# PravCoder/Multi-Modal-Medical-Imaging-and-Report-ML-Diagnosis-System

Measured on AMD Instinct MI355X. Metric: multimodal samples/sec (train fwd+bwd) at 1/2/4/8 MI355X; MFMA util %, higher is better.
Workload: dtype bf16; 1 GPU; C4: ResNet-50 + 2-layer BiLSTM, 128 samples/GPU (1024 global at 8 GPUs); image_tower=resnet50, text_tower=bilstm, global_batch=128, per_gpu_batch=128, seq_len=128, image_hw=224, parallelism=dp1

## Files before the change

### multi-modal-medical-imaging-and-report-ml-diagnosis-system_amd/csrc/capi.cpp

```cpp
#include <stdarg.h>
#include <stdio.h>
#include <stdlib.h>

#include <mutex>
#include <vector>

#include <hip/hip_ext.h>

#include "../../include/mmdx.h"
#include "common.h"

static thread_local char g_err[512] = "";

extern "C" void mmdx_set_error(const char* fmt, ...) {
  va_list ap;
  va_start(ap, fmt);
  vsnprintf(g_err, sizeof(g_err), fmt, ap);
  va_end(ap);
}

extern "C" const char* mmdx_last_error(void) { return g_err; }

extern "C" int mmdx_version(void) { return 1; }

namespace mmdx {

static long env_long(const char* name, long dflt) {
  const char* e = getenv(name);
  return e && *e ? atol(e) : dflt;
}

static Knobs read_knobs() {
  Knobs k;
  const long w = env_long("MMDX_CONV_N64_WIDE", -1);
  k.conv_n64_wide = w < 0 ? -1 : w == 0 ? 0 : 1;
  k.conv_8w128 = env_long("MMDX_CONV_8W128", 1) != 0;
  k.stem_direct = env_long("MMDX_STEM_DIRECT", 1) != 0;
  const long t = env_long("MMDX_WGRAD_TARGET", 256);
  k.wgrad_target = t >= 64 && t <= 4096 ? t : 256;
  k.wgrad_rq = env_long("MMDX_WGRAD_RQ", 1) != 0;
  k.gemm256_fwd_min = env_long("MMDX_GEMM256_FWD_MIN", 90);
  k.gemm_8w128 = env_long("MMDX_GEMM_8W128", 1) != 0;
  const long s = env_long("MMDX_SPLITK_TARGET", 256);
  k.splitk_target = s >= 64 ? s : 256;
  k.splitk_vec = env_long("MMDX_SPLITK_VEC", 1) != 0;
  k.wgrad_bias_fused = env_long("MMDX_WGRAD_BIAS_FUSED", 1) != 0;
  k.bias_grad_gemm = env_long("MMDX_BIAS_GRAD_GEMM", 0) == 1;
  k.ln_bwd_rpw = env_long("MMDX_LN_BWD_RPW", 8) == 4 ? 4 : 8;
  k.attn_fwd_nw = (int)env_long("MMDX_ATTN_FWD_NW", 0);
  k.attn_bwd_nw = (int)env_long("MMDX_ATTN_BWD_NW", 0);
  k.lstm_bwd_probe = env_long("MMDX_LSTM_BWD_PROBE", 0) != 0;
  k.bn_bwd_pair = env_long("MMDX_BN_BWD_PAIR", 1) != 0;
  return k;
}

static Knobs g_knobs;
static std::once_flag g_knobs_once;

const Knobs& knobs() {
  std::call_once(g_knobs_once, [] { g_knobs = read_knobs(); });
  return g_knobs;
}

}

extern "C" int mmdx_reload_config(void) {
  mmdx::knobs();
  mmdx::g_knobs = mmdx::read_knobs();
  return 0;
}

extern "C" int mmdx_bn_bwd_pair_enabled(void) { return mmdx::knobs().bn_bwd_pair ? 1 : 0; }

extern "C" int mmdx_stream_create(int priority, int cus, void** out) {
  MMDX_CHECK_ARG(out, "mmdx_stream_create: out is NULL");
  *out = nullptr;
  int dev = 0, n = 0;
  MMDX_CHECK_ARG(hipGetDevice(&dev) == hipSuccess &&
                     hipDeviceGetAttribute(&n, hipDeviceAttributeMultiprocessorCount, dev) ==
                         hipSuccess && n > 0,
                 "mmdx_stream_create: no device");
  hipStream_t s = nullptr;
  if (cus <= 0 || cus >= n) {
    MMDX_CHECK_ARG(hipStreamCreateWithPriority(&s, hipStreamNonBlocking, priority) == hipSuccess,
                   "mmdx_stream_create: hipStreamCreateWithPriority failed");
  } else {
    std::vector<uint32_t> mask((n + 31) / 32, 0u);
    for (int i = 0; i < cus; ++i) {
      const int cu = (int)((long)i * n / cus);
      mask[cu / 32] |= 1u << (cu % 32);
    }
    MMDX_CHECK_ARG(hipExtStreamCreateWithCUMask(&s, (uint32_t)mask.size(), mask.data()) ==
                       hipSuccess,
                   "mmdx_stream_create: hipExtStreamCreateWithCUMask failed");
  }
  *out = (void*)s;
  return 0;
}

extern "C" int mmdx_stream_destroy(void* s) {
  MMDX_CHECK_ARG(s && hipStreamDestroy((hipStream_t)s) == hipSuccess, "mmdx_stream_destroy");
  return 0;
}
```

### multi-modal-medical-imaging-and-report-ml-diagnosis-system_amd/csrc/common.h

```cpp
#pragma once
#include <hip/hip_runtime.h>

#include <algorithm>
#include <stdint.h>
#include <stddef.h>

namespace mmdx {

typedef __bf16 bf16;
typedef _Float16 f16;
typedef __attribute__((ext_vector_type(8))) __bf16 bf16x8;
typedef __attribute__((ext_vector_type(8))) _Float16 f16x8;
typedef __attribute__((ext_vector_type(4))) __bf16 bf16x4;
typedef __attribute__((ext_vector_type(4))) float f32x4;
typedef __attribute__((ext_vector_type(2))) float f32x2;
typedef __attribute__((ext_vector_type(16))) float f32x16;
typedef __attribute__((ext_vector_type(4))) unsigned int u32x4;
typedef __attribute__((ext_vector_type(4))) short s16x4;

enum Dtype { F32 = 0, BF16 = 1, F16 = 2 };
enum Act { ACT_NONE = 0, ACT_RELU = 1, ACT_GELU = 2, ACT_GELU_BWD = 3 };

constexpr int WAVE = 64;

struct Knobs {
  int conv_n64_wide;
  bool conv_8w128;
  bool stem_direct;
  long wgrad_target;
  bool wgrad_rq;
  long gemm256_fwd_min;
  bool gemm_8w128;
  long splitk_target;
  bool splitk_vec;
  bool wgrad_bias_fused;
  bool bias_grad_gemm;
  int ln_bwd_rpw;
  int attn_fwd_nw;
  int attn_bwd_nw;
  bool lstm_bwd_probe;
  bool bn_bwd_pair;
};
const Knobs& knobs();

__device__ __forceinline__ float to_f(float x) { return x; }
__device__ __forceinline__ float to_f(bf16 x) { return (float)x; }
__device__ __forceinline__ float to_f(f16 x) { return (float)x; }
template <typename T> __device__ __forceinline__ T from_f(float x);
template <> __device__ __forceinline__ float from_f<float>(float x) { return x; }
template <> __device__ __forceinline__ bf16 from_f<bf16>(float x) { return (bf16)x; }
template <> __device__ __forceinline__ f16 from_f<f16>(float x) { return (f16)x; }

template <typename T> struct Vec16;
template <> struct Vec16<bf16> { static constexpr int N = 8; typedef bf16x8 type; };
template <> struct Vec16<float> { static constexpr int N = 4; typedef f32x4 type; };
template <> struct Vec16<f16> { static constexpr int N = 8; typedef f16x8 type; };

#define MMDX_DISPATCH(dtype, ...)                  \
  do {                                             \
    if ((dtype) == ::mmdx::BF16) {                 \
      typedef ::mmdx::bf16 T;                      \
      __VA_ARGS__;                                 \
    } else if ((dtype) == ::mmdx::F16) {           \
      typedef ::mmdx::f16 T;                       \
      __VA_ARGS__;                                 \
    } else {                                       \
      typedef float T;                             \
      __VA_ARGS__;                                 \
    }                                              \
  } while (0)

__device__ __forceinline__ float gelu_erf(float x) {
  return 0.5f * x * (1.0f + erff(x * 0.70710678118654752f));
}
__device__ __forceinline__ float gelu_erf_grad(float x) {
  const float cdf = 0.5f * (1.0f + erff(x * 0.70710678118654752f));
  const float pdf = 0.39894228040143268f * __expf(-0.5f * x * x);
  return cdf + x * pdf;
}

__device__ __forceinline__ float wave_sum(float v) {
#pragma unroll
  for (int o = 32; o > 0; o >>= 1) v += __shfl_xor(v, o, 64);
  return v;
}
__device__ __forceinline__ float wave_max(float v) {
#pragma unroll
  for (int o = 32; o > 0; o >>= 1) v = fmaxf(v, __shfl_xor(v, o, 64));
  return v;
}

template <int NT>
__device__ __forceinline__ float block_sum(float v, float* red) {
  v = wave_sum(v);
  const int w = threadIdx.x >> 6, l = threadIdx.x & 63;
  if (l == 0) red[w] = v;
  __syncthreads();
  float t = 0.f;
#pragma unroll
  for (int i = 0; i < NT / 64; ++i) t += red[i];
  __syncthreads();
  return t;
}

static inline int grid_for(long n, int per = 256) {
  return (int)std::max<long>(1, std::min<long>((n + per - 1) / per, 8192));
}

#define GRID_STRIDE(i, n) \
  for (long i = blockIdx.x * (long)blockDim.x + threadIdx.x; i < (n); i += (long)gridDim.x * blockDim.x)

}

extern "C" void mmdx_set_error(const char* fmt, ...);

#define MMDX_CHECK_ARG(cond, ...)                     \
  do {                                               \
    if (!(cond)) {                                   \
      mmdx_set_error(__VA_ARGS__);                   \
      return -22;                       \
    }                                                \
  } while (0)

#define MMDX_LAUNCH_CHECK()                                          \
  do {                                                               \
    hipError_t _e = hipGetLastError();                               \
    if (_e != hipSuccess) {                                          \
      mmdx_set_error("HIP launch failed: %s", hipGetErrorString(_e)); \
      return -(int)_e;                                               \
    }                                                                \
  } while (0)
```

### multi-modal-medical-imaging-and-report-ml-diagnosis-system_amd/csrc/misc.hip

```cpp
#include <algorithm>

#include "common.h"
#include "dropout_rng.h"
#include "pool.h"
#include "../../include/mmdx.h"

namespace mmdx {

template <typename T>
__global__ void maxpool_fwd_kernel(const T* __restrict__ x, int N, int H, int W, int C, int k,
                                   int s, int p, T* __restrict__ y, uint8_t* __restrict__ am,
                                   int P, int Q) {
  typedef typename Vec16<T>::type V;
  constexpr int VEC = Vec16<T>::N;
  const int cv = C / VEC;
  const long total = (long)N * P * Q * cv;
  GRID_STRIDE(i, total) {
    const int c = (int)(i % cv) * VEC;
    long t = i / cv;
    const int q = (int)(t % Q); t /= Q;
    const int pp = (int)(t % P);
    const int n = (int)(t / P);
    float best[VEC];
    int arg[VEC];
// ... 4 lines not shown
      if ((unsigned)ih >= (unsigned)H) continue;
      for (int ss = 0; ss < k; ++ss) {
        const int iw = q * s - p + ss;
        if ((unsigned)iw >= (unsigned)W) continue;
        const V v = *(const V*)(x + (((long)n * H + ih) * W + iw) * C + c);
#pragma unroll
        for (int j = 0; j < VEC; ++j) {
          const float f = to_f(v[j]);
          if (arg[j] < 0 || f > best[j] || (f != f && best[j] == best[j])) {
            best[j] = f;
            arg[j] = r * k + ss;
          }
        }
      }
    }
    V o;
#pragma unroll
    for (int j = 0; j < VEC; ++j) {
      o[j] = from_f<T>(best[j]);
      am[i * VEC + j] = (uint8_t)arg[j];
    }
    *(V*)(y + i * VEC) = o;
  }
}

template <typename T>
__global__ void maxpool_bwd_kernel(const uint8_t* __restrict__ am, const T* __restrict__ dy,
                                   int N, int H, int W, int C, int k, int s, int p, int P, int Q,
                                   T* __restrict__ dx) {
  typedef typename Vec16<T>::type V;
  constexpr int VEC = Vec16<T>::N;
  const int cv = C / VEC;
  const long total = (long)N * H * W * cv;
  GRID_STRIDE(i, total) {
    const int c = (int)(i % cv) * VEC;
    long t = i / cv;
    const int w = (int)(t % W); t /= W;
    const int h = (int)(t % H);
    const int n = (int)(t / H);
    float acc[VEC];
#pragma unroll
    for (int j = 0; j < VEC; ++j) acc[j] = 0.f;
    const int p_lo = max(0, (h + p - k + s) / s), p_hi = min(P - 1, (h + p) / s);
    const int q_lo = max(0, (w + p - k + s) / s), q_hi = min(Q - 1, (w + p) / s);
    for (int pp = p_lo; pp <= p_hi; ++pp) {
      const int r = h + p - pp * s;
      if (r < 0 || r >= k) continue;
      for (int q = q_lo; q <= q_hi; ++q) {
        const int ss = w + p - q * s;
        if (ss < 0 || ss >= k) continue;
        const long o = (((long)n * P + pp) * Q + q) * C + c;
        const V g = *(const V*)(dy + o);
#pragma unroll
        for (int j = 0; j < VEC; ++j)
          if (am[o + j] == r * k + ss) acc[j] += to_f(g[j]);
      }
    }
    V out;
#pragma unroll
    for (int j = 0; j < VEC; ++j) out[j] = from_f<T>(acc[j]);
    *(V*)(dx + i * VEC) = out;
  }
}


__device__ __forceinline__ void bn_coef_fwd(const float* gamma, const float* beta,
                                            const float* mean, const float* rstd, int c,
                                            float& scale, float& shift) {
  const float g = gamma ? gamma[c] : 1.f;
  scale = g * rstd[c];
  shift = (beta ? beta[c] : 0.f) - mean[c] * g * rstd[c];
}

template <typename T, bool BN = false>
__global__ void maxpool3s2_fwd_kernel(const T* __restrict__ x, int N, int H, int W, int C,
                                      int p, T* __restrict__ y, uint8_t* __restrict__ am, int P,
                                      int Q, const float* __restrict__ gamma,
                                      const float* __restrict__ beta,
                                      const float* __restrict__ mean,
                                      const float* __restrict__ rstd, int relu) {
  typedef typename Vec16<T>::type V;
  constexpr int VEC = Vec16<T>::N;
  typedef typename ArgPack<VEC>::type A;
  const int cv = C / VEC;
  const long total = (long)N * P * Q * cv;
  const bool fixed_c = blockDim.x % cv == 0;
  float sc[VEC], sh[VEC];
  if constexpr (BN) {
    if (fixed_c) {
      const int c0 = (int)(threadIdx.x % cv) * VEC;
#pragma unroll
      for (int j = 0; j < VEC; ++j) bn_coef_fwd(gamma, beta, mean, rstd, c0 + j, sc[j], sh[j]);
    }
  }
  GRID_STRIDE(i, total) {
    const unsigned ui = (unsigned)i, ucv = (unsigned)cv;
    const int c = (int)(ui % ucv) * VEC;
    if constexpr (BN) {
      if (!fixed_c) {
#pragma unroll
        for (int j = 0; j < VEC; ++j) bn_coef_fwd(gamma, beta, mean, rstd, c + j, sc[j], sh[j]);
      }
    }
    unsigned t = ui / ucv;
    const int q = (int)(t % (unsigned)Q); t /= (unsigned)Q;
    const int pp = (int)(t % (unsigned)P);
    const int n = (int)(t / (unsigned)P);
    V v[9];
    bool ok[9];
#pragma unroll
    for (int r = 0; r < 3; ++r) {
      const int ih = pp * 2 - p + r;
#pragma unroll
      for (int ss = 0; ss < 3; ++ss) {
        const int iw = q * 2 - p + ss;
        ok[r * 3 + ss] = (unsigned)ih < (unsigned)H && (unsigned)iw < (unsigned)W;
        v[r * 3 + ss] = ok[r * 3 + ss] ? *(const V*)(x + (((long)n * H + ih) * W + iw) * C + c)
                                       : V{};
      }
    }
    float best[VEC];
    int arg[VEC];
#pragma unroll
    for (int j = 0; j < VEC; ++j) { best[j] = -INFINITY; arg[j] = -1; }
#pragma unroll
    for (int w9 = 0; w9 < 9; ++w9) {
      if (!ok[w9]) continue;
#pragma unroll
      for (int j = 0; j < VEC; ++j) {
        float f = to_f(v[w9][j]);
        if constexpr (BN) {
          f = f * sc[j] + sh[j];
          if (relu) f = fmaxf(f, 0.f);
          f = to_f(from_f<T>(f));
        }
        if (arg[j] < 0 || f > best[j] || (f != f && best[j] == best[j])) {
          best[j] = f;
          arg[j] = w9;
        }
      }
    }
    V o;
    A packed = 0;
#pragma unroll
    for (int j = 0; j < VEC; ++j) {
      o[j] = from_f<T>(best[j]);
      packed |= (A)(uint8_t)arg[j] << (8 * j);
    }
    *(A*)(am + i * VEC) = packed;
    *(V*)(y + i * VEC) = o;
  }
}

template <typename T>
__global__ void maxpool3s2_bwd_kernel(const uint8_t* __restrict__ am, const T* __restrict__ dy,
                                      int N, int H, int W, int C, int p, int P, int Q,
                                      T* __restrict__ dx) {
  typedef typename Vec16<T>::type V;
  constexpr int VEC = Vec16<T>::N;
  const Pool3s2Grad<T> pg{am, dy, H, W, C, p, P, Q};
  const int cv = C / VEC;
  const long total = (long)N * H * W * cv;
  GRID_STRIDE(i, total) {
    const unsigned ui = (unsigned)i, ucv = (unsigned)cv;
    const int c = (int)(ui % ucv) * VEC;
    unsigned t = ui / ucv;
    const int w = (int)(t % (unsigned)W); t /= (unsigned)W;
    const int h = (int)(t % (unsigned)H);
    const int n = (int)(t / (unsigned)H);
    *(V*)(dx + i * VEC) = pg.at(n, h, w, c);
  }
}

template <typename T>
__global__ void avgpool_fwd_kernel(const T* __restrict__ x, int N, int HW, int C,
                                   T* __restrict__ y) {
  const long total = (long)N * C;
  GRID_STRIDE(i, total) {
    const int c = (int)(i % C);
    const long n = i / C;
    float acc = 0.f;
    for (int k = 0; k < HW; ++k) acc += to_f(x[(n * HW + k) * C + c]);
    y[i] = from_f<T>(acc / (float)HW);
  }
}

template <typename T>
__global__ void avgpool_bwd_kernel(const T* __restrict__ dy, int N, int HW, int C,
                                   T* __restrict__ dx) {
  const long total = (long)N * HW * C;
  const float inv = 1.f / (float)HW;
  GRID_STRIDE(i, total) {
    const int c = (int)(i % C);
    const long n = i / ((long)HW * C);
    dx[i] = from_f<T>(to_f(dy[n * C + c]) * inv);
  }
}

template <typename T>
__global__ void nchw_to_nhwc_kernel(const float* __restrict__ x, int N, int C, int H, int W,
                                    int cp, T* __restrict__ y) {
  const long total = (long)N * H * W;
  GRID_STRIDE(i, total) {
    const long hw = i % ((long)H * W);
    const long n = i / ((long)H * W);
    for (int c = 0; c < cp; ++c)
      y[i * cp + c] = from_f<T>(c < C ? x[(n * C + c) * H * W + hw] : 0.f);
  }
}

template <typename D, typename S>
__global__ void cast_kernel(const S* __restrict__ x, long n, D* __restrict__ y) {
  GRID_STRIDE(i, n) y[i] = from_f<D>(to_f(x[i]));
}

__global__ void axpby_kernel(long n, float a, const float* __restrict__ x, float b,
                             const float* __restrict__ y, float* __restrict__ out) {
  GRID_STRIDE(i, n) out[i] = a * x[i] + (y ? b * y[i] : 0.f);
}

template <typename T>
__global__ void gelu_bwd_kernel(const T* __restrict__ pre, const T* __restrict__ dy, long n,
                                T* __restrict__ dx) {
  GRID_STRIDE(i, n) dx[i] = from_f<T>(to_f(dy[i]) * gelu_erf_grad(to_f(pre[i])));
}

constexpr int BG_ROWS = 256;
constexpr int BG_ROWS_MIN = 32;
static int bias_grad_rows(long M, int N, int vec) {
  const long nx = (N / vec + 63) / 64;
  const long nb_target = (1024 + nx - 1) / nx;
  long rows = (M + nb_target - 1) / nb_target;
  rows = (rows + 3) / 4 * 4;
  return (int)std::max<long>(BG_ROWS_MIN, std::min<long>(BG_ROWS, rows));
}
template <typename T>
__global__ __launch_bounds__(256) void bias_grad_partial_kernel(const T* __restrict__ dy,
                                                                long M, int N,
                                                                float* __restrict__ part,
                                                                int rows) {
  typedef typename Vec16<T>::type V;
  constexpr int VEC = Vec16<T>::N;
  __shared__ float red[4][64 * VEC];
  const int cv = threadIdx.x & 63, lane = threadIdx.x >> 6;
  const int j = blockIdx.x * 64 + cv;
  const bool ok = j < N / VEC;
  const long r0 = (long)blockIdx.y * rows, r1 = min(M, r0 + rows);
  float acc[VEC];
#pragma unroll
  for (int e = 0; e < VEC; ++e) acc[e] = 0.f;
  if (ok) {
#pragma unroll 4
    for (long r = r0 + lane; r < r1; r += 4) {
      const V v = ((const V*)(dy + r * N))[j];
#pragma unroll
      for (int e = 0; e < VEC; ++e) acc[e] += to_f(v[e]);
    }
  }
#pragma unroll
  for (int e = 0; e < VEC; ++e) red[lane][cv * VEC + e] = acc[e];
  __syncthreads();
  if (lane == 0 && ok) {
#pragma unroll
    for (int e = 0; e < VEC; ++e) {
      const int c = cv * VEC + e;
      part[(long)blockIdx.y * N + (long)j * VEC + e] =
          (red[0][c] + red[1][c]) + (red[2][c] + red[3][c]);
    }
  }
}
template <typename T>
__global__ void bias_grad_partial_scalar_kernel(const T* __restrict__ dy, long M, int N,
                                                float* __restrict__ part, int rows) {
  const int n = blockIdx.x * blockDim.x + threadIdx.x;
  if (n >= N) return;
  const long r0 = (long)blockIdx.y * rows, r1 = min(M, r0 + rows);
  float acc = 0.f;
  for (long r = r0; r < r1; ++r) acc += to_f(dy[r * N + n]);
  part[(long)blockIdx.y * N + n] = acc;
}
__global__ __launch_bounds__(256) void bias_grad_finalize_kernel(const float* __restrict__ part,
                                                                 int nb, int N, float* db,
                                                                 float beta_acc) {
  __shared__ float red[4][64];
  const int cc = threadIdx.x & 63, lane = threadIdx.x >> 6;
  const int n = blockIdx.x * 64 + cc;
  float acc = 0.f;
  if (n < N) {
#pragma unroll 4
    for (int b = lane; b < nb; b += 4) acc += part[(long)b * N + n];
  }
  red[lane][cc] = acc;
  __syncthreads();
  if (lane != 0 || n >= N) return;
  const float s = (red[0][cc] + red[1][cc]) + (red[2][cc] + red[3][cc]);
  db[n] = beta_acc != 0.f ? beta_acc * db[n] + s : s;
}

template <typename T>
__global__ void dropout_fwd_kernel(const T* __restrict__ x, long n, float p, uint64_t seed,
                                   uint64_t off, const uint64_t* __restrict__ ctr,
                                   T* __restrict__ y, uint8_t* __restrict__ mask) {
  const float scale = 1.f / (1.f - p);
  const uint64_t base = dropout_stream_base(seed, ctr) + off;
  GRID_STRIDE(i, n) {
    const uint8_t keep = dropout_keep(base, (uint64_t)i, p);
    mask[i] = keep;
    y[i] = from_f<T>(keep ? to_f(x[i]) * scale : 0.f);
  }
}
__global__ void counter_incr_kernel(uint64_t* c) { c[0] += 1; }
void dropout_counter_advance(uint64_t* counter, hipStream_t stream) {
  hipLaunchKernelGGL(counter_incr_kernel, dim3(1), dim3(1), 0, stream, counter);
}

template <typename T>
__global__ void dropout_bwd_kernel(const T* __restrict__ dy, const uint8_t* __restrict__ mask,
                                   long n, float p, T* __restrict__ dx) {
  const float scale = 1.f / (1.f - p);
  GRID_STRIDE(i, n) dx[i] = from_f<T>(mask[i] ? to_f(dy[i]) * scale : 0.f);
}

__global__ void bce_fwd_kernel(const float* __restrict__ z, const float* __restrict__ y, int n,
                               float* loss) {
  __shared__ float red[4];
  float acc = 0.f;
  for (int i = threadIdx.x; i < n; i += blockDim.x) {
    const float zi = z[i], yi = y[i];
    const float mx = fmaxf(-zi, 0.f);
    acc += (1.f - yi) * zi + mx + logf(expf(-mx) + expf(-zi - mx));
  }
  acc = block_sum<256>(acc, red);
  if (threadIdx.x == 0) loss[0] = acc / (float)n;
}
__global__ void bce_bwd_kernel(const float* __restrict__ z, const float* __restrict__ y, int n,
                               const float* __restrict__ dloss, float* __restrict__ dz) {
  const float g = (dloss ? dloss[0] : 1.f) / (float)n;
  for (int i = blockIdx.x * blockDim.x + threadIdx.x; i < n; i += gridDim.x * blockDim.x) {
    const float s = 1.f / (1.f + expf(-z[i]));
    dz[i] = (s - y[i]) * g;
  }
}

}

using namespace mmdx;

#define DISPATCH_T(dtype, ...) MMDX_DISPATCH(dtype, __VA_ARGS__)

extern "C" int mmdx_maxpool_fwd(int dtype, const void* x, int N, int H, int W, int C, int k,
                                int s, int p, void* y, uint8_t* argmax, int P, int Q,
                                void* stream) {
  const int VEC = dtype == F32 ? 4 : 8;
  MMDX_CHECK_ARG(C % VEC == 0 && k * k <= 255 && argmax, "maxpool: bad args");
  MMDX_CHECK_ARG(P == (H + 2 * p - k) / s + 1 && Q == (W + 2 * p - k) / s + 1,
                 "maxpool: inconsistent output size");
  const long total = (long)N * P * Q * (C / VEC);
  MMDX_CHECK_ARG((long)N * H * W * C < (1L << 31), "maxpool: more than 2^31 input elements");
  if (k == 3 && s == 2)
    DISPATCH_T(dtype, hipLaunchKernelGGL((maxpool3s2_fwd_kernel<T, false>),
                                         dim3(grid_for(total)), dim3(256), 0, (hipStream_t)stream,
                                         (const T*)x, N, H, W, C, p, (T*)y, argmax, P, Q,
                                         (const float*)nullptr, (const float*)nullptr,
                                         (const float*)nullptr, (const float*)nullptr, 0));
  else
    DISPATCH_T(dtype, hipLaunchKernelGGL(maxpool_fwd_kernel<T>, dim3(grid_for(total)),
                                         dim3(256), 0, (hipStream_t)stream, (const T*)x, N, H, W,
                                         C, k, s, p, (T*)y, argmax, P, Q));
  MMDX_LAUNCH_CHECK();
  return 0;
}

extern "C" int mmdx_maxpool_bn_fwd(int dtype, const void* x, int N, int H, int W, int C,
                                   int k, int s, int p, const float* gamma, const float* beta,
                                   const float* save_mean, const float* save_rstd, int relu,
                                   void* y, uint8_t* argmax, int P, int Q, void* stream) {
  const int VEC = dtype == F32 ? 4 : 8;
  MMDX_CHECK_ARG(C % VEC == 0 && argmax && save_mean && save_rstd, "maxpool bn: bad args");
  MMDX_CHECK_ARG(k == 3 && s == 2, "maxpool bn: only the 3x3 / stride-2 stem pool is fused");
  MMDX_CHECK_ARG(P == (H + 2 * p - k) / s + 1 && Q == (W + 2 * p - k) / s + 1,
                 "maxpool bn: inconsistent output size");
  const long total = (long)N * P * Q * (C / VEC);
  MMDX_CHECK_ARG((long)N * H * W * C < (1L << 31), "maxpool bn: more than 2^31 input elements");
  DISPATCH_T(dtype, hipLaunchKernelGGL((maxpool3s2_fwd_kernel<T, true>), dim3(grid_for(total)),
                                       dim3(256), 0, (hipStream_t)stream, (const T*)x, N, H, W, C,
                                       p, (T*)y, argmax, P, Q, gamma, beta, save_mean, save_rstd,
                                       relu));
  MMDX_LAUNCH_CHECK();
  return 0;
}

extern "C" int mmdx_maxpool_bwd(int dtype, const uint8_t* argmax, const void* dy, int N, int H,
                                int W, int C, int k, int s, int p, int P, int Q, void* dx,
                                void* stream) {
  const int VEC = dtype == F32 ? 4 : 8;
  MMDX_CHECK_ARG(C % VEC == 0, "maxpool bwd: bad C");
  const long total = (long)N * H * W * (C / VEC);
  MMDX_CHECK_ARG((long)N * H * W * C < (1L << 31), "maxpool bwd: more than 2^31 elements");
  if (k == 3 && s == 2 && p <= 1)
    DISPATCH_T(dtype, hipLaunchKernelGGL(maxpool3s2_bwd_kernel<T>, dim3(grid_for(total)),
                                         dim3(256), 0, (hipStream_t)stream, argmax,
                                         (const T*)dy, N, H, W, C, p, P, Q, (T*)dx));
  else
    DISPATCH_T(dtype, hipLaunchKernelGGL(maxpool_bwd_kernel<T>, dim3(grid_for(total)),
                                         dim3(256), 0, (hipStream_t)stream, argmax,
                                         (const T*)dy, N, H, W, C, k, s, p, P, Q, (T*)dx));
  MMDX_LAUNCH_CHECK();
  return 0;
}

extern "C" int mmdx_avgpool_fwd(int dtype, const void* x, int N, int HW, int C, void* y,
                                void* stream) {
  const long total = (long)N * C;
  DISPATCH_T(dtype, hipLaunchKernelGGL(avgpool_fwd_kernel<T>, dim3(grid_for(total)), dim3(256),
                                       0, (hipStream_t)stream, (const T*)x, N, HW, C, (T*)y));
  MMDX_LAUNCH_CHECK();
  return 0;
}

extern "C" int mmdx_avgpool_bwd(int dtype, const void* dy, int N, int HW, int C, void* dx,
                                void* stream) {
  const long total = (long)N * HW * C;
  DISPATCH_T(dtype, hipLaunchKernelGGL(avgpool_bwd_kernel<T>, dim3(grid_for(total)), dim3(256),
                                       0, (hipStream_t)stream, (const T*)dy, N, HW, C, (T*)dx));
  MMDX_LAUNCH_CHECK();
  return 0;
}

extern "C" int mmdx_nchw_to_nhwc(int dtype, const float* x, int N, int C, int H, int W,
                                 int c_pad, void* y, void* stream) {
  MMDX_CHECK_ARG(c_pad >= C, "nchw_to_nhwc: c_pad < C");
  const long total = (long)N * H * W;
  DISPATCH_T(dtype, hipLaunchKernelGGL(nchw_to_nhwc_kernel<T>, dim3(grid_for(total)), dim3(256),
                                       0, (hipStream_t)stream, x, N, C, H, W, c_pad, (T*)y));
  MMDX_LAUNCH_CHECK();
  return 0;
}

extern "C" int mmdx_cast(int dst, int src, const void* x, long n, void* y, void* stream) {
  hipStream_t st = (hipStream_t)stream;
  if (dst == BF16 && src == F32)
    hipLaunchKernelGGL((cast_kernel<bf16, float>), dim3(grid_for(n)), dim3(256), 0, st,
                       (const float*)x, n, (bf16*)y);
  else if (dst == F32 && src == BF16)
    hipLaunchKernelGGL((cast_kernel<float, bf16>), dim3(grid_for(n)), dim3(256), 0, st,
                       (const bf16*)x, n, (float*)y);
  else if (dst == F32 && src == F32)
    hipLaunchKernelGGL((cast_kernel<float, float>), dim3(grid_for(n)), dim3(256), 0, st,
                       (const float*)x, n, (float*)y);
  else if (dst == F16 && src == F32)
    hipLaunchKernelGGL((cast_kernel<f16, float>), dim3(grid_for(n)), dim3(256), 0, st,
                       (const float*)x, n, (f16*)y);
  else if (dst == F32 && src == F16)
    hipLaunchKernelGGL((cast_kernel<float, f16>), dim3(grid_for(n)), dim3(256), 0, st,
                       (const f16*)x, n, (float*)y);
  else
    hipLaunchKernelGGL((cast_kernel<bf16, bf16>), dim3(grid_for(n)), dim3(256), 0, st,
                       (const bf16*)x, n, (bf16*)y);
  MMDX_LAUNCH_CHECK();
  return 0;
}

extern "C" int mmdx_gelu_bwd(int dtype, const void* pre, const void* dy, long n, void* dx,
                             void* stream) {
  DISPATCH_T(dtype, hipLaunchKernelGGL(gelu_bwd_kernel<T>, dim3(grid_for(n)), dim3(256), 0,
                                       (hipStream_t)stream, (const T*)pre, (const T*)dy, n,
                                       (T*)dx));
  MMDX_LAUNCH_CHECK();
  return 0;
}

static bool bias_grad_gemm_ok(int dtype, long M, int N) {
  const bool on = knobs().bias_grad_gemm;
  return on && dtype != F32 && M % 8 == 0 && N % 8 == 0 && M < (1L << 30);
}
static size_t bias_grad_ones_bytes(long M) { return ((size_t)M * 2 + 255) & ~(size_t)255; }

template <typename T>
__global__ void fill_ones_kernel(T* __restrict__ p, long n) {
  GRID_STRIDE(i, n) p[i] = from_f<T>(1.f);
}

extern "C" size_t mmdx_bias_grad_workspace_size(long M, int N) {
  const size_t cs = (size_t)((M + BG_ROWS_MIN - 1) / BG_ROWS_MIN) * N * sizeof(float);
  const size_t gm = M < (1L << 30) ? bias_grad_ones_bytes(M) +
                                         mmdx_gemm_workspace_size(BF16, 1, N, (int)M)
                                   : 0;
  return std::max(cs, gm);
}

extern "C" int mmdx_bias_grad(int dtype, const void* dy, long M, int N, float* db,
                              float beta_acc, void* ws, size_t ws_bytes, void* stream) {
  if (bias_grad_gemm_ok(dtype, M, N) && ((uintptr_t)dy & 15) == 0 && ws &&
      ws_bytes >= mmdx_bias_grad_workspace_size(M, N)) {
    hipStream_t st = (hipStream_t)stream;
    char* ones = (char*)ws;
    const size_t ob = bias_grad_ones_bytes(M);
    DISPATCH_T(dtype, hipLaunchKernelGGL(fill_ones_kernel<T>, dim3(grid_for(M)), dim3(256), 0,
                                         st, (T*)ones, M));
    MMDX_LAUNCH_CHECK();
    return mmdx_gemm(dtype, 1, N, (int)M, ones, M, 1, dy, N, 0, db, N, F32, nullptr, nullptr,
                     0, 1.f, beta_acc, nullptr, ones + ob, ws_bytes - ob, stream);
  }
  const int vec = dtype == F32 ? 4 : 8;
  const int rows = bias_grad_rows(M, N, vec);
  const int nb = (int)((M + rows - 1) / rows);
  MMDX_CHECK_ARG(ws && ws_bytes >= mmdx_bias_grad_workspace_size(M, N),
                 "bias_grad: workspace too small");
  hipStream_t st = (hipStream_t)stream;
  if (N % vec == 0 && ((uintptr_t)dy & 15) == 0)
    DISPATCH_T(dtype, hipLaunchKernelGGL(bias_grad_partial_kernel<T>,
                                         dim3((N / vec + 63) / 64, nb), dim3(256), 0, st,
                                         (const T*)dy, M, N, (float*)ws, rows));
  else
    DISPATCH_T(dtype, hipLaunchKernelGGL(bias_grad_partial_scalar_kernel<T>,
                                         dim3((N + 255) / 256, nb), dim3(256), 0, st,
                                         (const T*)dy, M, N, (float*)ws, rows));
  hipLaunchKernelGGL(bias_grad_finalize_kernel, dim3((N + 63) / 64), dim3(256), 0, st,
                     (const float*)ws, nb, N, db, beta_acc);
  MMDX_LAUNCH_CHECK();
  return 0;
}

extern "C" int mmdx_dropout_fwd(int dtype, const void* x, long n, float p, uint64_t seed,
                                uint64_t offset, uint64_t* counter, void* y, uint8_t* mask,
                                void* stream) {
  MMDX_CHECK_ARG(p >= 0.f && p < 1.f, "dropout: p out of range");
  DISPATCH_T(dtype, hipLaunchKernelGGL(dropout_fwd_kernel<T>, dim3(grid_for(n)), dim3(256), 0,
                                       (hipStream_t)stream, (const T*)x, n, p, seed, offset,
                                       (const uint64_t*)counter, (T*)y, mask));
  if (counter) dropout_counter_advance(counter, (hipStream_t)stream);
  MMDX_LAUNCH_CHECK();
  return 0;
}

extern "C" int mmdx_dropout_bwd(int dtype, const void* dy, const uint8_t* mask, long n, float p,
                                void* dx, void* stream) {
  DISPATCH_T(dtype, hipLaunchKernelGGL(dropout_bwd_kernel<T>, dim3(grid_for(n)), dim3(256), 0,
                                       (hipStream_t)stream, (const T*)dy, mask, n, p, (T*)dx));
  MMDX_LAUNCH_CHECK();
// ... 29 lines not shown
```

### multi-modal-medical-imaging-and-report-ml-diagnosis-system_amd/csrc/norm.hip

```cpp
#include <algorithm>
#include <type_traits>
#include <cstdlib>

#include "common.h"
#include "dropout_rng.h"
#include "pool.h"
#include "../../include/mmdx.h"

namespace mmdx {

constexpr int BN_NT = 256;

struct BnLayout {
  int ct;
  int rt;
  int cgroups;
  int rblocks;
  long rows_per_block;
};

static BnLayout bn_layout(long rows, int C, int vec) {
  BnLayout L;
  const int cv = C / vec;
  L.ct = std::min(cv, 64);
// ... 50 lines not shown
        sum[j] += d;
        sq[j] += d * d;
      }
      ++cnt;
    }
  }
  const int me = ty * ct + tx;
  s_n[me] = (float)cnt;
#pragma unroll
  for (int j = 0; j < VEC; ++j) {
    const float m = cnt ? sum[j] / cnt : 0.f;
    s_mean[me * VEC + j] = piv[j] + m;
    s_m2[me * VEC + j] = cnt ? fmaxf(sq[j] - sum[j] * m, 0.f) : 0.f;
  }
  __syncthreads();
  if (ty == 0 && c0 < C) {
#pragma unroll
    for (int j = 0; j < VEC; ++j) {
      float n = 0.f, mean = 0.f, m2 = 0.f;
      for (int y = 0; y < rt; ++y) {
        const int o = y * ct + tx;
        chan_merge(n, mean, m2, s_n[o], s_mean[o * VEC + j], s_m2[o * VEC + j]);
      }
      part[(long)(c0 + j) * gridDim.x + blockIdx.x] = make_float2(mean, m2);
    }
  }
}

constexpr int FIN_W = 4;

template <int TPC, class F>
__device__ __forceinline__ float slab_sum(int nblk, int sub, float* red, F f) {
  float a4[4] = {0.f, 0.f, 0.f, 0.f};
  for (int b0 = sub; b0 < nblk; b0 += 4 * TPC) {
#pragma unroll
    for (int j = 0; j < 4; ++j) {
      const int b = b0 + TPC * j;
      if (b < nblk) a4[j] += f(b);
    }
  }
  const float v = (a4[0] + a4[1]) + (a4[2] + a4[3]);
  if constexpr (TPC == 64) return wave_sum(v);
  else return block_sum<256>(v, red);
}

template <int TPC, int PER, class F>
__device__ __forceinline__ float slab_sum_regs(const float2* vals, int nblk, int sub, float* red,
                                               F f) {
  float a4[4] = {0.f, 0.f, 0.f, 0.f};
#pragma unroll
  for (int j = 0; j < PER; ++j) {
    const int b = sub + TPC * j;
    if (b < nblk) a4[j & 3] += f(b, vals[j]);
  }
  const float v = (a4[0] + a4[1]) + (a4[2] + a4[3]);
  if constexpr (TPC == 64) return wave_sum(v);
  else return block_sum<256>(v, red);
}

constexpr int FIN_PER = 16;

struct BnFinArgs {
  const float2* part;
  int nblk;
  long rows, rpb;
  int C;
  const float* gamma;
  const float* beta;
  float* running_mean;
  float* running_var;
  float momentum, eps;
  float* save_mean;
  float* save_rstd;
  float* scale;
  float* shift;
};

template <int TPC>
__device__ __forceinline__ void bn_finalize_body(const BnFinArgs& a, int bid, float* red) {
  const int sub = threadIdx.x % TPC;
  const int c = bid * (256 / TPC) + threadIdx.x / TPC;
  if (c >= a.C) return;
  const int nblk = a.nblk;
  const long rows = a.rows, rpb = a.rpb;
  const long last = rows - (long)(nblk - 1) * rpb;
  const float2* pc = a.part + (long)c * nblk;
  float mean, m2;
  if (nblk <= TPC * FIN_PER) {
    float2 v[FIN_PER];
#pragma unroll
    for (int j = 0; j < FIN_PER; ++j) {
      const int b = sub + TPC * j;
      v[j] = b < nblk ? pc[b] : make_float2(0.f, 0.f);
    }
    mean = slab_sum_regs<TPC, FIN_PER>(v, nblk, sub, red, [&](int b, float2 p) {
      return (b == nblk - 1 ? (float)last : (float)rpb) * p.x;
    }) / (float)rows;
    m2 = slab_sum_regs<TPC, FIN_PER>(v, nblk, sub, red, [&](int b, float2 p) {
      const float d = p.x - mean;
      return p.y + (b == nblk - 1 ? (float)last : (float)rpb) * d * d;
    });
  } else {
    mean = slab_sum<TPC>(nblk, sub, red, [&](int b) {
      return (b == nblk - 1 ? (float)last : (float)rpb) * pc[b].x;
    }) / (float)rows;
    m2 = slab_sum<TPC>(nblk, sub, red, [&](int b) {
      const float2 p = pc[b];
      const float d = p.x - mean;
      return p.y + (b == nblk - 1 ? (float)last : (float)rpb) * d * d;
    });
  }
  if (sub != 0) return;
  const float var = m2 / (float)rows;
  const float rstd = rsqrtf(var + a.eps);
  a.save_mean[c] = mean;
  a.save_rstd[c] = rstd;
  if (a.running_mean) {
    const float unb = rows > 1 ? m2 / (float)(rows - 1) : var;
    a.running_mean[c] = (1.f - a.momentum) * a.running_mean[c] + a.momentum * mean;
    a.running_var[c] = (1.f - a.momentum) * a.running_var[c] + a.momentum * unb;
  }
  const float g = a.gamma ? a.gamma[c] : 1.f;
  a.scale[c] = g * rstd;
  a.shift[c] = (a.beta ? a.beta[c] : 0.f) - mean * g * rstd;
}

template <int TPC>
__global__ __launch_bounds__(256) void bn_finalize_kernel(BnFinArgs a) {
  __shared__ float red[4];
  bn_finalize_body<TPC>(a, blockIdx.x, red);
}

__global__ void bn_eval_coef_kernel(int C, const float* __restrict__ gamma,
                                    const float* __restrict__ beta, const float* rm,
                                    const float* rv, float eps, float* save_mean,
                                    float* save_rstd, float* scale, float* shift) {
  const int c = blockIdx.x * blockDim.x + threadIdx.x;
  if (c >= C) return;
  const float rstd = rsqrtf(rv[c] + eps);
  const float g = gamma ? gamma[c] : 1.f;
  save_mean[c] = rm[c];
  save_rstd[c] = rstd;
  scale[c] = g * rstd;
  shift[c] = (beta ? beta[c] : 0.f) - rm[c] * g * rstd;
}

struct RowTile { int cv, tpr, rpi; };
__host__ __device__ inline RowTile row_tile(int C, int vec) {
  RowTile t;
  t.cv = C / vec;
  t.tpr = t.cv < 256 ? t.cv : 256;
  t.rpi = 256 / t.tpr;
  return t;
}

template <int VEC>
__device__ __forceinline__ void load_coef(const float* p, float* out) {
#pragma unroll
  for (int e = 0; e < VEC; e += 4) {
    const f32x4 v = *(const f32x4*)(p + e);
    out[e] = v[0]; out[e + 1] = v[1]; out[e + 2] = v[2]; out[e + 3] = v[3];
  }
}

__device__ __forceinline__ void bn_coef(const float* gamma, const float* beta, float mean,
                                        float rstd, int c, float& scale, float& shift) {
  const float g = gamma ? gamma[c] : 1.f;
  scale = g * rstd;
  shift = (beta ? beta[c] : 0.f) - mean * g * rstd;
}

template <typename T>
__device__ __forceinline__ void bn_apply_vec(const typename Vec16<T>::type& v,
                                             const typename Vec16<T>::type& rr, bool has_res,
                                             const float* sc, const float* sh, int relu, long i,
                                             T* __restrict__ y, uint8_t* __restrict__ mask) {
  typedef typename Vec16<T>::type V;
  constexpr int VEC = Vec16<T>::N;
  V o;
#pragma unroll
  for (int e = 0; e < VEC; ++e) {
    float f = to_f(v[e]) * sc[e] + sh[e];
    if (has_res) f += to_f(rr[e]);
    if (relu) f = fmaxf(f, 0.f);
    o[e] = from_f<T>(f);
  }
  ((V*)y)[i] = o;
  if (mask) {
    unsigned b = 0;
#pragma unroll
    for (int e = 0; e < VEC; ++e) b |= (to_f(o[e]) > 0.f ? 1u : 0u) << e;
    mask[i] = (uint8_t)b;
  }
}

template <typename T>
__global__ __launch_bounds__(256) void bn_apply_kernel(const T* __restrict__ x,
                                                       const T* __restrict__ res, long rows,
                                                       int C, const float* __restrict__ scale,
                                                       const float* __restrict__ shift, int relu,
                                                       T* __restrict__ y,
                                                       uint8_t* __restrict__ mask) {
  typedef typename Vec16<T>::type V;
  constexpr int VEC = Vec16<T>::N;
  const RowTile rt = row_tile(C, VEC);
  const int j0 = threadIdx.x % rt.tpr, ro = threadIdx.x / rt.tpr;
  for (int j = j0; j < rt.cv; j += rt.tpr) {
    float sc[VEC], sh[VEC];
    load_coef<VEC>(scale + j * VEC, sc);
    load_coef<VEC>(shift + j * VEC, sh);
    for (long r = (long)blockIdx.x * rt.rpi + ro; r < rows; r += (long)gridDim.x * rt.rpi) {
      const long i = r * rt.cv + j;
      const V v = __builtin_nontemporal_load((const V*)x + i);
      V rr{};
      if (res) rr = __builtin_nontemporal_load((const V*)res + i);
      bn_apply_vec<T>(v, rr, res != nullptr, sc, sh, relu, i, y, mask);
    }
  }
}

template <typename T, class G, int MODE>
__global__ __launch_bounds__(BN_NT) void bn_bwd_reduce_kernel(
    const T* __restrict__ x, const T* __restrict__ y, const G dy, long rows, int C,
    int ct, long rpb, const float* __restrict__ mean, const float* __restrict__ rstd,
    const float* __restrict__ gamma, const float* __restrict__ bbeta, float2* __restrict__ part,
    const uint8_t* __restrict__ mask_k) {
  constexpr int relu = MODE != 0;
  const uint8_t* mask = MODE == 1 ? mask_k : nullptr;
  typedef typename Vec16<T>::type V;
  constexpr int VEC = Vec16<T>::N;
  __shared__ float s_a[BN_NT * VEC], s_b[BN_NT * VEC];
  const int tx = threadIdx.x % ct, ty = threadIdx.x / ct, rt = BN_NT / ct;
  const int c0 = (blockIdx.y * ct + tx) * VEC;
  const long r0 = blockIdx.x * rpb, r1 = min(rows, r0 + rpb);
  float sg[VEC], sgx[VEC], mu[VEC], rs[VEC], sc[VEC], sh[VEC];
  constexpr bool mask_x = MODE == 3;
#pragma unroll
  for (int j = 0; j < VEC; ++j) sg[j] = sgx[j] = mu[j] = rs[j] = sc[j] = sh[j] = 0.f;
  if (c0 < C) {
    load_coef<VEC>(mean + c0, mu);
    load_coef<VEC>(rstd + c0, rs);
    if constexpr (mask_x) {
      float ga[VEC], be[VEC];
      if (gamma) load_coef<VEC>(gamma + c0, ga);
      if (bbeta) load_coef<VEC>(bbeta + c0, be);
#pragma unroll
      for (int j = 0; j < VEC; ++j) {
        const float g = gamma ? ga[j] : 1.f;
        sc[j] = g * rs[j];
        sh[j] = (bbeta ? be[j] : 0.f) - mu[j] * g * rs[j];
      }
    }
  }
  if (c0 < C) {
    for (long r = r0 + ty; r < r1; r += rt) {
      const V vx = *(const V*)(x + r * C + c0);
      const V vd = dy.row(r, c0);
      V vy{};
      unsigned mb = 0;
      if (MODE == 1) mb = mask[r * (C / VEC) + c0 / VEC];
      else if (MODE == 2) vy = *(const V*)(y + r * C + c0);
#pragma unroll
      for (int j = 0; j < VEC; ++j) {
        float g = to_f(vd[j]);
        const float a = mask_x ? to_f(vx[j]) * sc[j] + sh[j] : to_f(vy[j]);
        const bool pos = MODE == 1 ? ((mb >> j) & 1u) != 0 : a > 0.f;
        if (relu && !pos) g = 0.f;
        sg[j] += g;
        sgx[j] += g * (to_f(vx[j]) - mu[j]) * rs[j];
      }
    }
  }
  const int me = ty * ct + tx;
#pragma unroll
  for (int j = 0; j < VEC; ++j) {
    s_a[me * VEC + j] = sg[j];
    s_b[me * VEC + j] = sgx[j];
  }
  __syncthreads();
  if (ty == 0 && c0 < C) {
#pragma unroll
    for (int j = 0; j < VEC; ++j) {
      float a = 0.f, b = 0.f;
      for (int yy = 0; yy < rt; ++yy) {
        a += s_a[(yy * ct + tx) * VEC + j];
        b += s_b[(yy * ct + tx) * VEC + j];
      }
      part[(long)(c0 + j) * gridDim.x + blockIdx.x] = make_float2(a, b);
    }
  }
}

struct BnBwdFinArgs {
  const float2* part;
  int nblk;
  long rows;
  int C, train;
  const float* gamma;
  const float* bbeta;
  const float* mean;
  const float* rstd;
  float* dgamma;
  float* dbeta;
  float beta_acc;
  float* coef;
};

template <int TPC>
__device__ __forceinline__ void bn_bwd_finalize_body(const BnBwdFinArgs& a, int bid,
                                                     float* red) {
  const int sub = threadIdx.x % TPC;
  const int c = bid * (256 / TPC) + threadIdx.x / TPC;
  const int C = a.C, nblk = a.nblk;
  if (c >= C) return;
  const float2* pc = a.part + (long)c * nblk;
// ... 919 lines not shown
```

Measured before the change: 10110 samples/s.

## Add row-reusing fast 3x3 stride-2 maxpool kernel for ResNet stem

Adds a new forward maxpool kernel for 3x3/stride-2 windows in which each thread computes a vertical strip of four output rows. The shared input row between adjacent output rows is kept in registers, so each output row needs only two new input rows instead of three. BN scale/shift coefficients are loaded once per thread as vectors, and 32-bit index math replaces 64-bit. The kernel is enabled by default behind an env knob, and load_coef is moved to common.h so both files can use it. The risks are a change in tie-breaking or argmax semantics at padded edges, and fewer threads available to hide latency.

Result: no change. 10150 samples/s (median of 6 runs) (+0.4%).

```diff
diff --git a/multi-modal-medical-imaging-and-report-ml-diagnosis-system_amd/csrc/capi.cpp b/multi-modal-medical-imaging-and-report-ml-diagnosis-system_amd/csrc/capi.cpp
--- a/multi-modal-medical-imaging-and-report-ml-diagnosis-system_amd/csrc/capi.cpp
+++ b/multi-modal-medical-imaging-and-report-ml-diagnosis-system_amd/csrc/capi.cpp
@@ -51,6 +51,7 @@
   k.attn_bwd_nw = (int)env_long("MMDX_ATTN_BWD_NW", 0);
   k.lstm_bwd_probe = env_long("MMDX_LSTM_BWD_PROBE", 0) != 0;
   k.bn_bwd_pair = env_long("MMDX_BN_BWD_PAIR", 1) != 0;
+  k.stem_pool_fast = env_long("MMDX_STEM_POOL_FAST", 1) != 0;
   return k;
 }
 
diff --git a/multi-modal-medical-imaging-and-report-ml-diagnosis-system_amd/csrc/common.h b/multi-modal-medical-imaging-and-report-ml-diagnosis-system_amd/csrc/common.h
--- a/multi-modal-medical-imaging-and-report-ml-diagnosis-system_amd/csrc/common.h
+++ b/multi-modal-medical-imaging-and-report-ml-diagnosis-system_amd/csrc/common.h
@@ -40,6 +40,7 @@
   int attn_bwd_nw;
   bool lstm_bwd_probe;
   bool bn_bwd_pair;
+  bool stem_pool_fast;
 };
 const Knobs& knobs();
 
@@ -55,6 +56,15 @@
 template <> struct Vec16<bf16> { static constexpr int N = 8; typedef bf16x8 type; };
 template <> struct Vec16<float> { static constexpr int N = 4; typedef f32x4 type; };
 template <> struct Vec16<f16> { static constexpr int N = 8; typedef f16x8 type; };
+
+template <int VEC>
+__device__ __forceinline__ void load_coef(const float* p, float* out) {
+#pragma unroll
+  for (int e = 0; e < VEC; e += 4) {
+    const f32x4 v = *(const f32x4*)(p + e);
+    out[e] = v[0]; out[e + 1] = v[1]; out[e + 2] = v[2]; out[e + 3] = v[3];
+  }
+}
 
 #define MMDX_DISPATCH(dtype, ...)                  \
   do {                                             \
diff --git a/multi-modal-medical-imaging-and-report-ml-diagnosis-system_amd/csrc/misc.hip b/multi-modal-medical-imaging-and-report-ml-diagnosis-system_amd/csrc/misc.hip
--- a/multi-modal-medical-imaging-and-report-ml-diagnosis-system_amd/csrc/misc.hip
+++ b/multi-modal-medical-imaging-and-report-ml-diagnosis-system_amd/csrc/misc.hip
@@ -180,6 +180,120 @@
   }
 }
 
+template <typename T, bool BN, bool RELU>
+__device__ __forceinline__ float pool_tap(T raw, float sc, float sh) {
+  float f = to_f(raw);
+  if constexpr (BN) {
+    f = f * sc + sh;
+    if (RELU) f = fmaxf(f, 0.f);
+    f = to_f(from_f<T>(f));
+  }
+  return f;
+}
+
+__device__ __forceinline__ void first_max(float& bv, int& bi, float f, int idx) {
+  const bool upd = !(f <= bv) & (bv == bv);
+  bv = upd ? f : bv;
+  bi = upd ? idx : bi;
+}
+
+template <typename T, bool BN, bool RELU>
+__device__ __forceinline__ void pool_row(const T* __restrict__ row, const int (&off)[3],
+                                         const int (&col)[3], const float* sc, const float* sh,
+                                         float* rv, int* rc) {
+  typedef typename Vec16<T>::type V;
+  constexpr int VEC = Vec16<T>::N;
+  V v[3];
+#pragma unroll
+  for (int ss = 0; ss < 3; ++ss) v[ss] = *(const V*)(row + off[ss]);
+#pragma unroll
+  for (int j = 0; j < VEC; ++j) {
+    rv[j] = pool_tap<T, BN, RELU>(v[0][j], sc[j], sh[j]);
+    rc[j] = col[0];
+    first_max(rv[j], rc[j], pool_tap<T, BN, RELU>(v[1][j], sc[j], sh[j]), col[1]);
+    first_max(rv[j], rc[j], pool_tap<T, BN, RELU>(v[2][j], sc[j], sh[j]), col[2]);
+  }
+}
+
+template <typename T, bool BN, bool RELU, int TP>
+__global__ __launch_bounds__(256) __attribute__((amdgpu_waves_per_eu(6))) void
+maxpool3s2_fwd_fast_kernel(
+    const T* __restrict__ x, int H, int W, int C, int p, T* __restrict__ y,
+    uint8_t* __restrict__ am, int P, int Q, int PC, unsigned total,
+    const float* __restrict__ gamma, const float* __restrict__ beta,
+    const float* __restrict__ mean, const float* __restrict__ rstd) {
+  typedef typename Vec16<T>::type V;
+  constexpr int VEC = Vec16<T>::N;
+  typedef typename ArgPack<VEC>::type A;
+  const unsigned i = blockIdx.x * 256u + threadIdx.x;
+  if (i >= total) return;
+  const unsigned ucv = (unsigned)(C / VEC);
+  const int c = (int)(i % ucv) * VEC;
+  unsigned t = i / ucv;
+  const int q = (int)(t % (unsigned)Q); t /= (unsigned)Q;
+  const int pp0 = (int)(t % (unsigned)PC) * TP;
+  const int n = (int)(t / (unsigned)PC);
+  float sc[VEC], sh[VEC];
+  if constexpr (BN) {
+    float ga[VEC], be[VEC], mu[VEC], rs[VEC];
+    load_coef<VEC>(mean + c, mu);
+    load_coef<VEC>(rstd + c, rs);
+    if (gamma) load_coef<VEC>(gamma + c, ga);
+    if (beta) load_coef<VEC>(beta + c, be);
+#pragma unroll
+    for (int j = 0; j < VEC; ++j) {
+      const float g = gamma ? ga[j] : 1.f;
+      sc[j] = g * rs[j];
+      sh[j] = (beta ? be[j] : 0.f) - mu[j] * g * rs[j];
+    }
+  } else {
+#pragma unroll
+    for (int j = 0; j < VEC; ++j) sc[j] = sh[j] = 0.f;
+  }
+  const T* xn = x + (long)n * H * W * C + c;
+  const int iw0 = 2 * q - p;
+  int off[3], col[3];
+#pragma unroll
+  for (int ss = 0; ss < 3; ++ss) {
+    col[ss] = (unsigned)(iw0 + ss) < (unsigned)W ? ss : 1;
+    off[ss] = (iw0 + col[ss]) * C;
+  }
+  const int rowC = W * C;
+  int ih = 2 * pp0 - p;
+  int base0 = ih < 0 ? 3 : 0;
+  float cv[VEC];
+  int cc[VEC];
+  pool_row<T, BN, RELU>(xn + (ih < 0 ? ih + 1 : ih) * rowC, off, col, sc, sh, cv, cc);
+  long o = (((long)n * P + pp0) * Q + q) * C + c;
+#pragma unroll 1
+  for (int k = 0; k < TP && pp0 + k < P; ++k, ih += 2, o += (long)Q * C) {
+    const bool ok2 = ih + 2 < H;
+    const int base2 = ok2 ? 6 : 3;
+    float rv[VEC];
+    int rc[VEC];
+    pool_row<T, BN, RELU>(xn + (ih + 1) * rowC, off, col, sc, sh, rv, rc);
+#pragma unroll
+    for (int j = 0; j < VEC; ++j) {
+      cc[j] += base0;
+      first_max(cv[j], cc[j], rv[j], rc[j] + 3);
+    }
+    pool_row<T, BN, RELU>(xn + (ok2 ? ih + 2 : ih + 1) * rowC, off, col, sc, sh, rv, rc);
+    V ov;
+    A packed = 0;
+#pragma unroll
+    for (int j = 0; j < VEC; ++j) {
+      first_max(cv[j], cc[j], rv[j], rc[j] + base2);
+      ov[j] = from_f<T>(cv[j]);
+      packed |= (A)(unsigned)cc[j] << (8 * j);
+      cv[j] = rv[j];
+      cc[j] = rc[j];
+    }
+    base0 = 0;
+    *(A*)(am + o) = packed;
+    *(V*)(y + o) = ov;
+  }
+}
+
 template <typename T>
 __global__ void maxpool3s2_bwd_kernel(const uint8_t* __restrict__ am, const T* __restrict__ dy,
                                       int N, int H, int W, int C, int p, int P, int Q,
@@ -376,6 +490,27 @@
 
 #define DISPATCH_T(dtype, ...) MMDX_DISPATCH(dtype, __VA_ARGS__)
 
+constexpr int POOL_TP = 4;
+
+template <typename T, bool BN>
+static void maxpool3s2_fwd_fast(const void* x, int N, int H, int W, int C, int p, void* y,
+                                uint8_t* argmax, int P, int Q, const float* gamma,
+                                const float* beta, const float* mean, const float* rstd, int relu,
+                                hipStream_t st) {
+  const int PC = (P + POOL_TP - 1) / POOL_TP;
+  const long total = (long)N * PC * Q * (C / Vec16<T>::N);
+  const dim3 g((unsigned)((total + 255) / 256));
+  if (g.x == 0) return;
+  if (BN && relu)
+    hipLaunchKernelGGL((maxpool3s2_fwd_fast_kernel<T, BN, BN, POOL_TP>), g, dim3(256), 0, st,
+                       (const T*)x, H, W, C, p, (T*)y, argmax, P, Q, PC, (unsigned)total, gamma,
+                       beta, mean, rstd);
+  else
+    hipLaunchKernelGGL((maxpool3s2_fwd_fast_kernel<T, BN, false, POOL_TP>), g, dim3(256), 0, st,
+                       (const T*)x, H, W, C, p, (T*)y, argmax, P, Q, PC, (unsigned)total, gamma,
+                       beta, mean, rstd);
+}
+
 extern "C" int mmdx_maxpool_fwd(int dtype, const void* x, int N, int H, int W, int C, int k,
                                 int s, int p, void* y, uint8_t* argmax, int P, int Q,
                                 void* stream) {
@@ -385,7 +520,11 @@
                  "maxpool: inconsistent output size");
   const long total = (long)N * P * Q * (C / VEC);
   MMDX_CHECK_ARG((long)N * H * W * C < (1L << 31), "maxpool: more than 2^31 input elements");
-  if (k == 3 && s == 2)
+  if (k == 3 && s == 2 && p <= 1 && knobs().stem_pool_fast)
+    DISPATCH_T(dtype, (maxpool3s2_fwd_fast<T, false>(x, N, H, W, C, p, y, argmax, P, Q, nullptr,
+                                                     nullptr, nullptr, nullptr, 0,
+                                                     (hipStream_t)stream)));
+  else if (k == 3 && s == 2)
     DISPATCH_T(dtype, hipLaunchKernelGGL((maxpool3s2_fwd_kernel<T, false>),
                                          dim3(grid_for(total)), dim3(256), 0, (hipStream_t)stream,
                                          (const T*)x, N, H, W, C, p, (T*)y, argmax, P, Q,
@@ -410,10 +549,15 @@
                  "maxpool bn: inconsistent output size");
   const long total = (long)N * P * Q * (C / VEC);
   MMDX_CHECK_ARG((long)N * H * W * C < (1L << 31), "maxpool bn: more than 2^31 input elements");
-  DISPATCH_T(dtype, hipLaunchKernelGGL((maxpool3s2_fwd_kernel<T, true>), dim3(grid_for(total)),
-                                       dim3(256), 0, (hipStream_t)stream, (const T*)x, N, H, W, C,
-                                       p, (T*)y, argmax, P, Q, gamma, beta, save_mean, save_rstd,
-                                       relu));
+  if (p <= 1 && knobs().stem_pool_fast)
+    DISPATCH_T(dtype, (maxpool3s2_fwd_fast<T, true>(x, N, H, W, C, p, y, argmax, P, Q, gamma, beta,
+                                                    save_mean, save_rstd, relu,
+                                                    (hipStream_t)stream)));
+  else
+    DISPATCH_T(dtype, hipLaunchKernelGGL((maxpool3s2_fwd_kernel<T, true>),
+                                         dim3(grid_for(total)), dim3(256), 0, (hipStream_t)stream,
+                                         (const T*)x, N, H, W, C, p, (T*)y, argmax, P, Q, gamma,
+                                         beta, save_mean, save_rstd, relu));
   MMDX_LAUNCH_CHECK();
   return 0;
 }
diff --git a/multi-modal-medical-imaging-and-report-ml-diagnosis-system_amd/csrc/norm.hip b/multi-modal-medical-imaging-and-report-ml-diagnosis-system_amd/csrc/norm.hip
--- a/multi-modal-medical-imaging-and-report-ml-diagnosis-system_amd/csrc/norm.hip
+++ b/multi-modal-medical-imaging-and-report-ml-diagnosis-system_amd/csrc/norm.hip
@@ -226,15 +226,6 @@
   t.tpr = t.cv < 256 ? t.cv : 256;
   t.rpi = 256 / t.tpr;
   return t;
-}
-
-template <int VEC>
-__device__ __forceinline__ void load_coef(const float* p, float* out) {
-#pragma unroll
-  for (int e = 0; e < VEC; e += 4) {
-    const f32x4 v = *(const f32x4*)(p + e);
-    out[e] = v[0]; out[e + 1] = v[1]; out[e + 2] = v[2]; out[e + 3] = v[3];
-  }
 }
 
 __device__ __forceinline__ void bn_coef(const float* gamma, const float* beta, float mean,
```
